# zssjh/stereo-semantic-vo

Measured on AMD Instinct MI355X. Metric: stereo frames/sec on KITTI 00 (full Tracking::Track chain), higher is better.
Workload: dtype u8; 1 GPU; BASELINE configs[2]: synth-kitti00 sequence of 4541 distinct 1241x376 stereo pairs, full Tracking::Track loop per frame (ORB on L and R, sparse stereo, matching passes 1+2, PnP-RANSAC, pose-only LM, map-point lifecycle); ONE sequence per GPU in strict frame order (replicas across GPUs); parallelism=one GPU, resident_pairs_per_gpu=4541, resident_input_bytes_per_gpu=4370984960, frames_tracked=4541, tracker_capacity_flag=0, pnp_samples_through_sequential_fallback=0

## Files before the change

stereo-semantic-vo_amd/csrc/svo_pose_dev.h:

```cpp
#pragma once
#include "svo_internal.h"
#include "svo_wave.h"

struct Se3 { double q[4]; double t[3]; };

__device__ __forceinline__ double pose_ndiv(double a, double b) {
  double r = __builtin_amdgcn_rcp(b);
  double e = __builtin_fma(-b, r, 1.0);
  r = __builtin_fma(r, e, r);
  e = __builtin_fma(-b, r, 1.0);
  r = __builtin_fma(r, e, r);
  const double q = a * r;
  const double rem = __builtin_fma(-b, q, a);
  return __builtin_fma(rem, r, q);
}
__device__ __forceinline__ double pose_rcp_refined(double b) {
  double r = __builtin_amdgcn_rcp(b);
  double e = __builtin_fma(-b, r, 1.0);
  r = __builtin_fma(r, e, r);
  e = __builtin_fma(-b, r, 1.0);
  r = __builtin_fma(r, e, r);
  return r;
}
__device__ __forceinline__ double pose_ndiv_r(double a, double b, double r) {
// ... 575 lines not shown
#include "svo_epnp_ord_dev.h"

struct PnpHyp {
  double R[9], t[3];
  int32_t cnt, ok;
};

__device__ __forceinline__ bool pnp_inlier(const double* R, const double* t, const double* X, const double* uv, const double* K) {
  double x = R[0] * X[0] + R[1] * X[1] + R[2] * X[2] + t[0];
  double y = R[3] * X[0] + R[4] * X[1] + R[5] * X[2] + t[1];
  double z = R[6] * X[0] + R[7] * X[1] + R[8] * X[2] + t[2];
  z = z != 0.0 ? 1. / z : 1.;
  x *= z; y *= z;
  const float px = (float)(x * K[0] + K[2]), py = (float)(y * K[1] + K[3]);
  const float dx = (float)uv[0] - px, dy = (float)uv[1] - py;
  const float err = dx * dx + dy * dy;
  return err <= 64.0f;
}

__device__ __forceinline__ void pnp_hyp_block(EpnpWaveLds* ws, const double* Xw, const double* uv, int n, const double* K,
                                              const uint16_t* subset, PnpHyp* out, int hyp_base) {
  const int lane = threadIdx.x & 63, wv = threadIdx.x >> 6;
  const int k = hyp_base + wv;
  if (k >= PNP_HYP) return;
  if (lane < 5) {
    const int e = min((int)subset[5 * k + lane], n - 1);
    ws[wv].x5[3 * lane] = Xw[3 * e]; ws[wv].x5[3 * lane + 1] = Xw[3 * e + 1]; ws[wv].x5[3 * lane + 2] = Xw[3 * e + 2];
    ws[wv].u5[2 * lane] = uv[2 * e]; ws[wv].u5[2 * lane + 1] = uv[2 * e + 1];
  }
  double R[9], t[3];
  const bool ok = epnp5_wave(ws[wv], K, R, t);
  int cnt = 0;
  if (ok)
    for (int e = lane; e < n; e += 64) cnt += pnp_inlier(R, t, Xw + 3 * e, uv + 2 * e, K) ? 1 : 0;
  cnt = wave_sum_i32_dpp(cnt);
  if (lane == 0) {
    PnpHyp h;
#pragma unroll
    for (int i = 0; i < 9; ++i) h.R[i] = R[i];
    h.t[0] = t[0]; h.t[1] = t[1]; h.t[2] = t[2];
    h.cnt = cnt; h.ok = ok ? 1 : 0;
    out[k] = h;
  }
}

struct PnpExactLds { epnp_exact::Work W; double R[9], t[3]; int ok; };
__device__ __forceinline__ void pnp_hyp_exact_wave(PnpExactLds& S, const double* Xw, const double* uv, int n, const double* K,
                                                   const uint16_t* subset, PnpHyp* out, int k) {
  const int lane = threadIdx.x & 63;
  if (k >= PNP_HYP) return;
  if (lane == 0) {
    double* x5 = S.W.PW0;
    double* u5 = S.W.gA;
    for (int i = 0; i < 5; ++i) {
      const int e = min((int)subset[5 * k + i], n - 1);
      x5[3 * i] = Xw[3 * e]; x5[3 * i + 1] = Xw[3 * e + 1]; x5[3 * i + 2] = Xw[3 * e + 2];
      u5[2 * i] = uv[2 * e]; u5[2 * i + 1] = uv[2 * e + 1];
    }
    S.ok = epnp_exact::solve5(S.W, x5, u5, K, S.R, S.t, nullptr) ? 1 : 0;
  }
  __builtin_amdgcn_fence(__ATOMIC_ACQ_REL, "workgroup");
  __builtin_amdgcn_wave_barrier();
  double R[9], t[3];
#pragma unroll
  for (int i = 0; i < 9; ++i) R[i] = S.R[i];
#pragma unroll
  for (int i = 0; i < 3; ++i) t[i] = S.t[i];
  const bool ok = S.ok != 0;
  int cnt = 0;
  if (ok)
    for (int e = lane; e < n; e += 64) cnt += pnp_inlier(R, t, Xw + 3 * e, uv + 2 * e, K) ? 1 : 0;
  cnt = wave_sum_i32_dpp(cnt);
  if (lane == 0) {
    PnpHyp h;
#pragma unroll
    for (int i = 0; i < 9; ++i) h.R[i] = R[i];
    h.t[0] = t[0]; h.t[1] = t[1]; h.t[2] = t[2];
    h.cnt = cnt; h.ok = ok ? 1 : 0;
    out[k] = h;
  }
}

struct PnpOrdLds { epnp_ord::Lds S; epnp_exact::Work W; };
template <bool AGENT_OUT = false>
__device__ __forceinline__ void pnp_hyp_ord_wave(PnpOrdLds& L, const double* Xw, const double* uv, int n, const double* K,
                                                 const uint16_t* subset, PnpHyp* out, int k, bool force_seq = false,
                                                 unsigned* word = nullptr ) {
  const int lane = threadIdx.x & 63;
  if (k >= PNP_HYP) return;
  if (lane < 5) {
    const int e = min((int)subset[5 * k + lane], n - 1);
    L.S.pws[3 * lane] = Xw[3 * e]; L.S.pws[3 * lane + 1] = Xw[3 * e + 1]; L.S.pws[3 * lane + 2] = Xw[3 * e + 2];
    L.S.us[2 * lane] = uv[2 * e]; L.S.us[2 * lane + 1] = uv[2 * e + 1];
  }
  double R[9], t[3];
  const bool ok = epnp_ord::solve5_wave(L.S, L.W, K, R, t, nullptr, force_seq);
  int cnt = 0;
  if (ok)
    for (int e = lane; e < n; e += 64) cnt += pnp_inlier(R, t, Xw + 3 * e, uv + 2 * e, K) ? 1 : 0;
  cnt = wave_sum_i32_dpp(cnt);
  if (lane == 0) {
    if (word) *word = (ok ? 0x80000000u : 0u) | (unsigned)cnt;
    if (AGENT_OUT) {
      PnpHyp* o = out + k;
#pragma unroll
      for (int i = 0; i < 9; ++i) __hip_atomic_store(reinterpret_cast<long long*>(&o->R[i]), __builtin_bit_cast(long long, R[i]), __ATOMIC_RELAXED, __HIP_MEMORY_SCOPE_AGENT);
#pragma unroll
      for (int i = 0; i < 3; ++i) __hip_atomic_store(reinterpret_cast<long long*>(&o->t[i]), __builtin_bit_cast(long long, t[i]), __ATOMIC_RELAXED, __HIP_MEMORY_SCOPE_AGENT);
      __hip_atomic_store(&o->cnt, cnt, __ATOMIC_RELAXED, __HIP_MEMORY_SCOPE_AGENT);
      __hip_atomic_store(&o->ok, ok ? 1 : 0, __ATOMIC_RELAXED, __HIP_MEMORY_SCOPE_AGENT);
    } else {
      PnpHyp h;
#pragma unroll
      for (int i = 0; i < 9; ++i) h.R[i] = R[i];
      h.t[0] = t[0]; h.t[1] = t[1]; h.t[2] = t[2];
      h.cnt = cnt; h.ok = ok ? 1 : 0;
      out[k] = h;
    }
  }
}

__device__ __forceinline__ int pnp_update_iters(double ep, int maxIters) {
  const double p = 0.99;
  ep = fmax(ep, 0.); ep = fmin(ep, 1.);
  double num = fmax(1. - p, 2.2250738585072014e-308);
  double denom = 1. - pow(1. - ep, 5.0);
  if (denom < 2.2250738585072014e-308) return 0;
  num = log(num);
  denom = log(denom);
  return denom >= 0 || -num >= maxIters * (-denom) ? maxIters : (int)rint(num / denom);
}

__device__ __forceinline__ int pnp_bound_after(const int* cnt, const int* ok, int n, int m) {
  int niters = PNP_HYP, maxGood = 0;
  if (n == 5) return 1;
  for (int iter = 0; iter < m && iter < niters; ++iter) {
    if (!ok[iter]) continue;
    const int g = cnt[iter];
    if (g > max(maxGood, 4)) { maxGood = g; niters = pnp_update_iters((double)(n - g) / n, niters); }
  }
  return niters;
}

__device__ __forceinline__ void pnp_update_terms(int g, int n, double* ld, int* r) {
  double ep = (double)(n - g) / n;
  ep = fmax(ep, 0.); ep = fmin(ep, 1.);
  const double denom = 1. - pow(1. - ep, 5.0);
  if (denom < 2.2250738585072014e-308) { *ld = 1.0; *r = 0; return; }
  const double num = log(fmax(1. - 0.99, 2.2250738585072014e-308));
  *ld = log(denom);
  *r = *ld < 0 ? (int)rint(num / *ld) : 0;
}
__device__ __forceinline__ int pnp_select_pre(const int* cnt, const int* ok, const double* ld, const int* r, int n, int* good, int* iters) {
  int niters = PNP_HYP, maxGood = 0, best = -1, run = 0;
  if (n == 5) {
    *good = ok[0] ? 5 : 0; *iters = 1;
    return ok[0] ? 0 : -1;
  }
  const double num = log(fmax(1. - 0.99, 2.2250738585072014e-308));
  for (int iter = 0; iter < niters; ++iter) {
    ++run;
    if (!ok[iter]) continue;
    const int g = cnt[iter];
    if (g > max(maxGood, 4)) {
      maxGood = g; best = iter;
      const double d = ld[iter];
      if (d == 1.0) niters = 0;
      else niters = d >= 0 || -num >= niters * (-d) ? niters : r[iter];
    }
  }
  *good = maxGood; *iters = run;
  return best;
}

__device__ __forceinline__ int pnp_select_pre_bound(const int* cnt, const int* ok, const double* ld, const int* r, int n, int m) {
  int niters = PNP_HYP, maxGood = 0;
  if (n == 5) return 1;
  const double num = log(fmax(1. - 0.99, 2.2250738585072014e-308));
  int iter = 0;
  for (; iter < niters; ++iter) {
    if (iter >= m) return m + 1;
    if (!ok[iter]) continue;
    const int g = cnt[iter];
    if (g > max(maxGood, 4)) {
      maxGood = g;
      const double d = ld[iter];
      if (d == 1.0) niters = 0;
      else niters = d >= 0 || -num >= niters * (-d) ? niters : r[iter];
    }
  }
  return iter;
}

__device__ __forceinline__ int pnp_select_pre_early(const int* cnt, const int* ok, const double* ld, const int* r, int n, int m,
                                                    int* best_out, int* good) {
  int niters = PNP_HYP, maxGood = 0, best = -1;
  if (n == 5) {
    *good = ok[0] ? 5 : 0; *best_out = ok[0] ? 0 : -1;
    return 1;
  }
  const double num = log(fmax(1. - 0.99, 2.2250738585072014e-308));
// ... 35 lines not shown
```

stereo-semantic-vo_amd/csrc/svo_track.hip:

```cpp
#include <chrono>
#include <cstddef>
#include <initializer_list>
#include <string>
#include <vector>
#include <algorithm>
#include <cstring>
#include <mutex>

#include "svo_internal.h"
#include "svo_wave.h"
#include "svo_gate.h"
#include "svo_pose_dev.h"
#include "svo_fmat_dev.h"

#define TRK_MAXKP 512
#define TRK_CAP 4096
#define TRK_ROWS_MAX 3072
#define TRK_LCAP 8
#define TRK_GPOS (1 << 20)
#define TRK_DNC 24
#define TRK_DENSE 0xFF

struct TrackPool {
  alignas(16) uint32_t desc[TRK_CAP * 8];
  int32_t create_id[TRK_CAP];
  int32_t gid[TRK_CAP];
  uint8_t bad[TRK_CAP];
  uint8_t in_local[TRK_CAP];
};

#define TP_EARLY 8
#define TP_FLAGS 16
struct TrackWork {
  int32_t ready;
  int32_t frame_id, nkp, n_stereo, n_pass1, n_pass2, n_new, n_local, skip_match;
  long long ts[8];
  long long rt[6];
  int32_t diag[2];
  int32_t n_edges;
  int32_t edge_gid[TRK_MAXKP];
  int32_t edge_kp[TRK_MAXKP];
  int32_t new_gid[TRK_MAXKP];
  int32_t pnp_best, pnp_iterations, pnp_inliers, pnp_ok;
  double T_pnp[16];
  int32_t hyp_done, pad_hyp;
  long long hyp_early[TP_FLAGS];
  long long hyp_rt[TP_EARLY];
};

struct TrackState {
  int32_t frame_num, npool, lastN, cur;
  int32_t next_gid, overflow, n_vetoed, n_boxes;
  int32_t epnp_fallbacks, pad_counters[3];
  int32_t last_mp[TRK_MAXKP];
  int32_t dbg_cur_mp[TRK_MAXKP];
  svo_camera cam;
  int32_t boxes[SVO_MAX_BOXES * 4];
  double F[9];
  float last_xy[TRK_MAXKP * 2];
  alignas(16) uint32_t last_desc[TRK_MAXKP * 8];
  int32_t bf_idx[TRK_MAXKP], bf_dist[TRK_MAXKP], bf_min;
  uint8_t bf_keep[TRK_MAXKP];
  float lastTcw[16];
  double Xw[TRK_MAXKP * 3], obs[TRK_MAXKP * 2], K[4], Tprior[16], T[16];
  svo_lm_stats lm;
  svo_pnp_stats pnp;
  PnpHyp hyp[PNP_HYP];
  long long pose_ts[16];
  TrackPool pool[2];
  uint16_t rowmin[TRK_CAP];
  uint8_t ncand[TRK_CAP];
  uint32_t cand[(size_t)TRK_CAP * 2 * TRK_LCAP];
  uint16_t D[(size_t)TRK_CAP * 512];
  float gpos[(size_t)TRK_GPOS * 3];
};

__device__ __forceinline__ int tk_wave_incl_scan(int v) {
  v += __builtin_amdgcn_update_dpp(0, v, 0x111, 0xf, 0xf, false);
  v += __builtin_amdgcn_update_dpp(0, v, 0x112, 0xf, 0xf, false);
  v += __builtin_amdgcn_update_dpp(0, v, 0x114, 0xf, 0xf, false);
  v += __builtin_amdgcn_update_dpp(0, v, 0x118, 0xf, 0xf, false);
  v += __builtin_amdgcn_update_dpp(0, v, 0x142, 0xa, 0xf, false);
  v += __builtin_amdgcn_update_dpp(0, v, 0x143, 0xc, 0xf, false);
  return v;
}
__device__ __forceinline__ int block_excl_scan(int v, int* sm , int* total) {
  const int lane = threadIdx.x & 63, wv = threadIdx.x >> 6;
  const int incl = tk_wave_incl_scan(v);
  const int nw = blockDim.x >> 6;
  __syncthreads();
  if (lane == 63) sm[wv] = incl;
  __syncthreads();
  const int4 a = reinterpret_cast<const int4*>(sm)[0], b = reinterpret_cast<const int4*>(sm)[1],
             c = reinterpret_cast<const int4*>(sm)[2], d = reinterpret_cast<const int4*>(sm)[3];
  const int t[16] = {a.x, a.y, a.z, a.w, b.x, b.y, b.z, b.w, c.x, c.y, c.z, c.w, d.x, d.y, d.z, d.w};
  int off = 0, tot = 0;
#pragma unroll
  for (int w = 0; w < 16; ++w) {
    off += w < wv ? t[w] : 0;
    tot += w < nw ? t[w] : 0;
  }
  *total = tot;
  return off + incl - v;
}

__device__ __forceinline__ void tk_unproject(const svo_camera& cam, float u, float v, float z,
                                             const float* Rwc, const float* twc, float* xyz) {
  const float x = (u - cam.cx) * z * (1 / cam.fx);
  const float y = (v - cam.cy) * z * (1 / cam.fy);
#pragma unroll
  for (int r = 0; r < 3; ++r) {
    const double acc = (double)Rwc[3 * r] * (double)x + (double)Rwc[3 * r + 1] * (double)y +
                       (double)Rwc[3 * r + 2] * (double)z;
    xyz[r] = (float)(acc + (double)twc[r]);
  }
}

__device__ __forceinline__ int ld_agent(const int* p) { return __hip_atomic_load(p, __ATOMIC_RELAXED, __HIP_MEMORY_SCOPE_AGENT); }
__device__ __forceinline__ long long ld_agent(const long long* p) { return __hip_atomic_load(p, __ATOMIC_RELAXED, __HIP_MEMORY_SCOPE_AGENT); }
__device__ __forceinline__ void st_agent(int* p, int v) { __hip_atomic_store(p, v, __ATOMIC_RELAXED, __HIP_MEMORY_SCOPE_AGENT); }
__device__ __forceinline__ void st_agent(long long* p, long long v) { __hip_atomic_store(p, v, __ATOMIC_RELAXED, __HIP_MEMORY_SCOPE_AGENT); }
#define TP_STORES_DONE() asm volatile("s_waitcnt vmcnt(0)" ::: "memory")
__device__ __forceinline__ long long tp_early_word(int frame_tag, unsigned ok_cnt) { return (long long)(((unsigned long long)(unsigned)frame_tag << 32) | ok_cnt); }
__device__ __forceinline__ int tp_early_tag(long long w) { return (int)((unsigned long long)w >> 32); }
__device__ __forceinline__ int tp_early_cnt(long long w) { return (int)((unsigned)w & 0x7fffffffu); }
__device__ __forceinline__ int tp_early_ok(long long w) { return (int)(((unsigned)w >> 31) & 1u); }

template <int ROWS>
__global__ __launch_bounds__(256) void k_ti_lists(TrackState* st, const uint32_t* desc, const int32_t* nkp_p, int kstride,
                                                  int lcap, int nblk) {
// ... 761 lines not shown
      if (s_lost) atomicOr(&st->overflow, 4);
    }
    __syncthreads();
    __builtin_amdgcn_fence(__ATOMIC_ACQUIRE, "agent");
    if (s_lost) return false;
  }
  return true;
}

#define TP_HYP_FIRST 16
#define TP_HYP_PRE 32
struct TpHypLds {
  double Xw[TRK_MAXKP * 3], uv[TRK_MAXKP * 2];
  EpnpWaveLds ws[4];
  int cnt[TP_HYP_PRE], ok[TP_HYP_PRE], bound;
};

__global__ __launch_bounds__(256) void k_tp_hyp(TrackState* st, const TrackWork* work, const svo_kp* kp, const uint16_t* subsets,
                                                int kstride, int hyp_base, int tag) {
  TpHypLds& S = *reinterpret_cast<TpHypLds*>(tk_smem);
  st += blockIdx.y; work += blockIdx.y; kp += (size_t)blockIdx.y * kstride;
  if (!tp_wait_work(st, work, tag)) return;
  const long long t_start = clock64();
  if (hyp_base == 0 && blockIdx.x == 0 && threadIdx.x == 0) const_cast<TrackWork*>(work)->rt[2] = wall_clock64();
  const int n = ld_agent(&work->n_edges), skip0 = ld_agent(&work->skip_match);
  const int gid0 = ld_agent(&work->edge_gid[threadIdx.x]), j0 = min(max(ld_agent(&work->edge_kp[threadIdx.x]), 0), kstride - 1);
  if (skip0 || n < 5) return;
  const int first = hyp_base + (int)blockIdx.x * (int)(blockDim.x >> 6);
  if (hyp_base > 0) {
    const int pre = min(hyp_base, TP_HYP_PRE);
    if ((int)threadIdx.x < pre) { S.cnt[threadIdx.x] = st->hyp[threadIdx.x].cnt; S.ok[threadIdx.x] = st->hyp[threadIdx.x].ok; }
    __syncthreads();
    if (threadIdx.x == 0) S.bound = pnp_bound_after(S.cnt, S.ok, n, pre);
    __syncthreads();
    if (first >= S.bound) return;
  }
  const float* gpos = st->gpos;
  for (int e = threadIdx.x; e < n; e += blockDim.x) {
    const bool first_e = e == (int)threadIdx.x;
    const float* gp = gpos + 3 * (size_t)((first_e ? gid0 : ld_agent(&work->edge_gid[e])) & (TRK_GPOS - 1));
    const svo_kp k = kp[first_e ? j0 : ld_agent(&work->edge_kp[e])];
    S.Xw[3 * e] = (double)gp[0]; S.Xw[3 * e + 1] = (double)gp[1]; S.Xw[3 * e + 2] = (double)gp[2];
    S.uv[2 * e] = (double)k.x; S.uv[2 * e + 1] = (double)k.y;
  }
  __syncthreads();
  const double K[4] = {(double)st->cam.fx, (double)st->cam.fy, (double)st->cam.cx, (double)st->cam.cy};
  const long long t_gather = clock64();
  pnp_hyp_block(S.ws, S.Xw, S.uv, n, K, subsets + (size_t)min(n, 512) * 500, st->hyp, first);
  if (first == 0 && threadIdx.x == 0) {
    st->pose_ts[0] = t_start; st->pose_ts[1] = t_gather; st->pose_ts[2] = S.ws[0].stamp[0]; st->pose_ts[3] = S.ws[0].stamp[4];
    st->pose_ts[4] = clock64();
    st->pose_ts[5] = S.ws[0].stamp[1]; st->pose_ts[6] = S.ws[0].stamp[2]; st->pose_ts[7] = S.ws[0].stamp[3]; st->pose_ts[12] = S.ws[0].sweeps;
    st->pose_ts[13] = S.ws[0].stamp[5]; st->pose_ts[14] = S.ws[0].stamp[6]; st->pose_ts[15] = S.ws[0].stamp[7];
  }
}

struct TpHypExactLds { double Xw[TRK_MAXKP * 3], uv[TRK_MAXKP * 2]; PnpExactLds ex; };
__global__ __launch_bounds__(64) void k_tp_hyp_exact(TrackState* st, TrackWork* work, const svo_kp* kp, const uint16_t* subsets,
                                                     int kstride, int tag) {
  TpHypExactLds& S = *reinterpret_cast<TpHypExactLds*>(tk_smem);
  st += blockIdx.y; work += blockIdx.y; kp += (size_t)blockIdx.y * kstride;
  if (!tp_wait_work(st, work, tag)) return;
  if (threadIdx.x == 0 && blockIdx.x == 0) work->rt[2] = wall_clock64();
  const int n = ld_agent(&work->n_edges);
  if (ld_agent(&work->skip_match) || n < 5) return;
  const float* gpos = st->gpos;
  for (int e = threadIdx.x; e < n; e += blockDim.x) {
    const float* gp = gpos + 3 * (size_t)(ld_agent(&work->edge_gid[e]) & (TRK_GPOS - 1));
    const svo_kp k = kp[ld_agent(&work->edge_kp[e])];
    S.Xw[3 * e] = (double)gp[0]; S.Xw[3 * e + 1] = (double)gp[1]; S.Xw[3 * e + 2] = (double)gp[2];
    S.uv[2 * e] = (double)k.x; S.uv[2 * e + 1] = (double)k.y;
  }
  __syncthreads();
  const double K[4] = {(double)st->cam.fx, (double)st->cam.fy, (double)st->cam.cx, (double)st->cam.cy};
  pnp_hyp_exact_wave(S.ex, S.Xw, S.uv, n, K, subsets + (size_t)min(n, 512) * 500, st->hyp, blockIdx.x);
}

struct TpHypOrdLds { double Xw[TRK_MAXKP * 3], uv[TRK_MAXKP * 2]; PnpOrdLds ord; int cnt[TP_HYP_PRE], ok[TP_HYP_PRE], bound; };
template <bool FUSED>
__device__ __forceinline__ void tp_hyp_ord_body(TpHypOrdLds& S, TrackState* st, TrackWork* work, const svo_kp* kp, const uint16_t* subsets,
                                                int kstride, int hyp_base, int sample, int tag, int force_seq, int semi = 0) {
  if (!tp_wait_work(st, work, tag)) return;
  const long long t_start = clock64();
  if (threadIdx.x == 0 && sample == 0) work->rt[2] = wall_clock64();
  const int n = ld_agent(&work->n_edges);
  const int frame_tag = FUSED ? ld_agent(&work->frame_id) + 1 : 0;
  if (ld_agent(&work->skip_match) || n < 5) return;
  if (FUSED && (force_seq >> 8) == sample + 1) return;
  if (FUSED && semi > 0) {
    const int tid = threadIdx.x;
    if (tid < semi) { S.cnt[tid] = ld_agent(&st->hyp[tid].cnt); S.ok[tid] = ld_agent(&st->hyp[tid].ok); }
    __syncthreads();
    if (tid == 0) S.bound = pnp_bound_after(S.cnt, S.ok, n, semi);
    __syncthreads();
    bool leave = sample >= S.bound;
    if (!leave && sample >= 2 * semi) {
      if (tid >= semi && tid < 2 * semi) {
        int spins = 0;
        long long w = 0;
        while (tp_early_tag(w = ld_agent(&work->hyp_early[tid])) != frame_tag && spins < (1 << 22)) { __builtin_amdgcn_s_sleep(2); ++spins; }
        const bool late = spins >= (1 << 22);
        S.cnt[tid] = late ? 0 : tp_early_cnt(w); S.ok[tid] = late ? 0 : tp_early_ok(w);
      }
      __syncthreads();
      if (tid == 0) S.bound = pnp_bound_after(S.cnt, S.ok, n, 2 * semi);
      __syncthreads();
      leave = sample >= S.bound;
    }
    if (leave) {
      if (tid == 0) {
        if (sample < TP_FLAGS) st_agent(&work->hyp_early[sample], tp_early_word(frame_tag, 0u));
        __hip_atomic_fetch_add(&work->hyp_done, 1, __ATOMIC_RELAXED, __HIP_MEMORY_SCOPE_AGENT);
      }
      return;
    }
  }
  if (hyp_base > 0) {
    const int pre = min(hyp_base, TP_HYP_PRE);
    if ((int)threadIdx.x < pre) { S.cnt[threadIdx.x] = st->hyp[threadIdx.x].cnt; S.ok[threadIdx.x] = st->hyp[threadIdx.x].ok; }
    __syncthreads();
    if (threadIdx.x == 0) S.bound = pnp_bound_after(S.cnt, S.ok, n, pre);
    __syncthreads();
    if (sample >= S.bound) return;
  }
  const float* gpos = st->gpos;
  for (int e = threadIdx.x; e < n; e += 64) {
    const float* gp = gpos + 3 * (size_t)(ld_agent(&work->edge_gid[e]) & (TRK_GPOS - 1));
    const svo_kp k = kp[ld_agent(&work->edge_kp[e])];
    S.Xw[3 * e] = (double)gp[0]; S.Xw[3 * e + 1] = (double)gp[1]; S.Xw[3 * e + 2] = (double)gp[2];
    S.uv[2 * e] = (double)k.x; S.uv[2 * e + 1] = (double)k.y;
  }
  __syncthreads();
  const double K[4] = {(double)st->cam.fx, (double)st->cam.fy, (double)st->cam.cx, (double)st->cam.cy};
  if (!FUSED && sample == 0) {
    for (int i = threadIdx.x; i < 3 * n; i += 64) st->Xw[i] = S.Xw[i];
    for (int i = threadIdx.x; i < 2 * n; i += 64) st->obs[i] = S.uv[i];
    if (threadIdx.x < 4) st->K[threadIdx.x] = K[threadIdx.x];
  }
  const long long t_gather = clock64();
  unsigned ok_cnt = 0;
  pnp_hyp_ord_wave<FUSED>(S.ord, S.Xw, S.uv, n, K, subsets + (size_t)min(n, 512) * 500, st->hyp, sample, (force_seq & 0xff) != 0, &ok_cnt);
  if (FUSED) {
    if (threadIdx.x == 0 && sample < TP_EARLY) st_agent(&work->hyp_rt[sample], (long long)wall_clock64());
    TP_STORES_DONE();
    if (threadIdx.x == 0) {
      if (sample < TP_FLAGS) st_agent(&work->hyp_early[sample], tp_early_word(frame_tag, ok_cnt));
      __hip_atomic_fetch_add(&work->hyp_done, 1, __ATOMIC_RELAXED, __HIP_MEMORY_SCOPE_AGENT);
    }
  }
  if (threadIdx.x == 0 && S.ord.S.flag) atomicAdd(&st->epnp_fallbacks, 1);
  if (sample == 0 && threadIdx.x == 0) {
    const long long* sp = S.ord.S.stamp;
    st->pose_ts[0] = t_start; st->pose_ts[1] = t_gather; st->pose_ts[2] = sp[0]; st->pose_ts[3] = sp[7];
    st->pose_ts[4] = clock64();
    st->pose_ts[5] = sp[2]; st->pose_ts[6] = sp[3]; st->pose_ts[7] = sp[4]; st->pose_ts[12] = S.ord.S.flag;
    st->pose_ts[13] = sp[4]; st->pose_ts[14] = sp[5]; st->pose_ts[15] = sp[6];
  }
}
__global__ __launch_bounds__(64) void k_tp_hyp_ord(TrackState* st, TrackWork* work, const svo_kp* kp, const uint16_t* subsets,
                                                   int kstride, int hyp_base, int tag, int force_seq) {
  TpHypOrdLds& S = *reinterpret_cast<TpHypOrdLds*>(tk_smem);
  st += blockIdx.y; work += blockIdx.y; kp += (size_t)blockIdx.y * kstride;
  tp_hyp_ord_body<false>(S, st, work, kp, subsets, kstride, hyp_base, hyp_base + (int)blockIdx.x, tag, force_seq);
}
__global__ __launch_bounds__(64) void k_tp_hyp_ord_first(TrackState* st, TrackWork* work, const svo_kp* kp, const uint16_t* subsets,
                                                         int kstride, int tag, int force_seq) {
  TpHypOrdLds& S = *reinterpret_cast<TpHypOrdLds*>(tk_smem);
  st += blockIdx.y; work += blockIdx.y; kp += (size_t)blockIdx.y * kstride;
  tp_hyp_ord_body<true>(S, st, work, kp, subsets, kstride, 0, (int)blockIdx.x, tag, force_seq);
}

struct TpLds {
  PoseLds pose;
  alignas(16) int sm[16];
  int cnt[PNP_HYP], ok[PNP_HYP], upd_r[PNP_HYP], best, good, iters;
  long long hrt[TP_EARLY];
  double tab_ld[PNP_MAXN + 1]; int tab_r[PNP_MAXN + 1];
  double pre_T[TP_EARLY][16]; Se3 pre_est[TP_EARLY];
  double T_end[16];
  long long t_samples, t_build;
  int late[TP_EARLY], lost;
  int recf[8];
  double upd_ld[PNP_HYP];
};

#define TPF_NT 256
template <bool FUSED>
__device__ __forceinline__ void tp_frame_body(TpLds& S, TrackState* st, TrackWork* work, const svo_kp* kp, const float* depth,
                                              svo_track_result* res_out, int kstride, int use_mfma, int tag, int pre_gathered) {
  const int tid = threadIdx.x;
  if (!tp_wait_work(st, work, tag)) return;
  if (!FUSED && tid == 0) work->rt[4] = wall_clock64();
  const long long tf0 = clock64();
  const int id = ld_agent(&work->frame_id), nkp = ld_agent(&work->nkp), skip = ld_agent(&work->skip_match), n_edges = ld_agent(&work->n_edges);
  const int gid0 = ld_agent(&work->edge_gid[tid]), j0 = min(max(ld_agent(&work->edge_kp[tid]), 0), kstride - 1);
  float* gpos = st->gpos;
  if (tid >= 64 && tid < 71) {
    const int* src = tid == 64 ? &work->n_stereo : tid == 65 ? &work->n_pass1 : tid == 66 ? &work->n_pass2 : tid == 67 ? &work->n_new
                   : tid == 68 ? &work->n_local : tid == 69 ? &work->diag[0] : &work->diag[1];
    S.recf[tid - 64] = ld_agent(src);
  }
  constexpr int NEWS = (TRK_MAXKP + TPF_NT - 1) / TPF_NT;
  int new_g[NEWS]; svo_kp new_k[NEWS]; float new_d[NEWS];
#pragma unroll
  for (int q = 0; q < NEWS; ++q) {
    const int j = tid + q * TPF_NT;
    new_g[q] = ld_agent(&work->new_gid[min(j, TRK_MAXKP - 1)]);
    new_k[q] = kp[min(j, kstride - 1)];
    new_d[q] = depth[min(j, kstride - 1)];
  }
  const bool have_corr = pre_gathered && !skip && n_edges >= 5 && id != 0;
  for (int e = tid; e < (have_corr ? 0 : n_edges); e += TPF_NT) {
    const int j = e == tid ? j0 : ld_agent(&work->edge_kp[e]);
    const svo_kp k = kp[j];
    float* gp = gpos + 3 * (size_t)((e == tid ? gid0 : ld_agent(&work->edge_gid[e])) & (TRK_GPOS - 1));
    float xyz[3];
    if (id == 0) {
      const float I3[9] = {1, 0, 0, 0, 1, 0, 0, 0, 1}, z3[3] = {0, 0, 0};
      tk_unproject(st->cam, k.x, k.y, depth[j], I3, z3, xyz);
      gp[0] = xyz[0]; gp[1] = xyz[1]; gp[2] = xyz[2];
    } else {
      xyz[0] = gp[0]; xyz[1] = gp[1]; xyz[2] = gp[2];
    }
    st->Xw[3 * e] = (double)xyz[0]; st->Xw[3 * e + 1] = (double)xyz[1]; st->Xw[3 * e + 2] = (double)xyz[2];
    st->obs[2 * e] = (double)k.x; st->obs[2 * e + 1] = (double)k.y;
    if (FUSED && e < POSE_CHUNK) {
      double* c5 = S.pose.tw + 5 * e;
      c5[0] = (double)xyz[0]; c5[1] = (double)xyz[1]; c5[2] = (double)xyz[2]; c5[3] = (double)k.x; c5[4] = (double)k.y;
    }
  }
  if (tid < 4 && !have_corr) st->K[tid] = (double)((const float*)&st->cam)[tid];
  const bool ran = !skip && n_edges >= 5;
  bool decided_early = false;
  double first[10] = {0, 0, 0, 0, 0, 0, 0, 0, 0, 0};
  if (FUSED) {
    if (tid < 4) S.pose.K[tid] = (double)((const float*)&st->cam)[tid];
    if (ran) {
      if (n_edges > 5)
        for (int g = 5 + tid; g <= n_edges; g += TPF_NT) {
          double ld; int r;
          pnp_update_terms(g, n_edges, &ld, &r);
          S.tab_ld[g] = ld; S.tab_r[g] = r;
        }
      if (tid >= TP_EARLY && tid < PNP_HYP) { S.cnt[tid] = 0; S.ok[tid] = 0; S.upd_ld[tid] = 1.0; S.upd_r[tid] = 0; }
    }
    __syncthreads();
    pose_edge_regs(S.pose.tw, S.pose.tw + 3, max(min(n_edges, POSE_CHUNK), 1), first, 5, 5);
  }
  if (FUSED && ran) {
    long long hp[12], hclk = 0;
    bool late = false;
    if (tid < TP_EARLY) {
      int spins = 0;
      long long w = 0;
      while (tp_early_tag(w = ld_agent(&work->hyp_early[tid])) != id + 1 && spins < (1 << 22)) { __builtin_amdgcn_s_sleep(1); ++spins; }
      late = spins >= (1 << 22);
      if (late) atomicOr(&st->overflow, 4);
      const PnpHyp& h = st->hyp[tid];
#pragma unroll
      for (int i = 0; i < 12; ++i) hp[i] = ld_agent(reinterpret_cast<const long long*>(i < 9 ? &h.R[i] : &h.t[i - 9]));
      hclk = ld_agent(&work->hyp_rt[tid]);
      S.late[tid] = late ? 1 : 0;
      const int c = late ? 0 : tp_early_cnt(w), o = late ? 0 : tp_early_ok(w);
      S.cnt[tid] = c; S.ok[tid] = o;
      const bool bound = o && c > 4 && n_edges > 5;
      const int g = min(max(c, 5), max(n_edges, 5));
      S.upd_ld[tid] = bound ? S.tab_ld[g] : 1.0; S.upd_r[tid] = bound ? S.tab_r[g] : 0;
    }
    __syncthreads();
    if (tid == 64) {
      int l = 0;
      for (int k = 0; k < TP_EARLY; ++k) l |= S.late[k];
      S.lost = l;
      int best = -1, good = 0;
      S.iters = l ? 0 : pnp_select_pre_early(S.cnt, S.ok, S.upd_ld, S.upd_r, n_edges, TP_EARLY, &best, &good);
      S.best = best; S.good = good;
    }
    if (tid < TP_EARLY) {
      double Tp[16];
#pragma unroll
      for (int q = 0; q < 16; ++q) {
        const int r = q >> 2, c = q & 3;
        Tp[q] = r == 3 ? (c == 3 ? 1.0 : 0.0) : __builtin_bit_cast(double, c == 3 ? hp[9 + r] : hp[3 * r + c]);
        S.pre_T[tid][q] = Tp[q];
      }
      Se3 e0;
      pose_start_estimate(Tp, 1, e0);
      S.pre_est[tid] = e0;
      S.hrt[tid] = late ? 0 : hclk;
    }
    __syncthreads();
    decided_early = S.lost || S.iters <= TP_EARLY;
    if (!decided_early) {
      if (tid == 0) {
        int spins = 0;
        while (ld_agent(&work->hyp_done) < PNP_HYP && spins < (1 << 22)) { __builtin_amdgcn_s_sleep(1); ++spins; }
        if (spins >= (1 << 22)) { atomicOr(&st->overflow, 4); S.lost = 1; }
      }
      __syncthreads();
    }
  } else if (tid == 0) {
    S.lost = 0;
  }
  if (FUSED && tid == 0) S.t_samples = wall_clock64();
  const bool fast = FUSED && ran && decided_early;
  if (!fast) {
    if (ran && !decided_early && !(FUSED && S.lost))
      for (int h = tid; h < PNP_HYP; h += TPF_NT) {
        const int c = FUSED ? ld_agent(&st->hyp[h].cnt) : st->hyp[h].cnt, o = FUSED ? ld_agent(&st->hyp[h].ok) : st->hyp[h].ok;
        S.cnt[h] = c; S.ok[h] = o;
        double ld = 1.0; int r = 0;
        if (o && c > 4 && n_edges > 5) pnp_update_terms(c, n_edges, &ld, &r);
        S.upd_ld[h] = ld; S.upd_r[h] = r;
      }
    __syncthreads();
    if (tid == 0) {
      int good = 0, iters = 0;
      S.best = (ran && !S.lost) ? pnp_select_pre(S.cnt, S.ok, S.upd_ld, S.upd_r, n_edges, &good, &iters) : -1;
      S.good = good; S.iters = iters;
    }
    __syncthreads();
  }
  const int tb = FUSED ? TPF_NT - 64 : 0;
  if (tid >= tb && tid < tb + 16) {
    const int q = tid - tb;
    double v;
    if (S.best >= 0) {
      const PnpHyp& h = st->hyp[S.best];
      const int r = q >> 2, c = q & 3;
      if (fast) {
        v = S.pre_T[S.best][q];
      } else if (FUSED) {
        const double* src = r == 3 ? nullptr : (c == 3 ? &h.t[r] : &h.R[3 * r + c]);
        v = src ? __builtin_bit_cast(double, ld_agent(reinterpret_cast<const long long*>(src))) : (c == 3 ? 1.0 : 0.0);
      } else {
        v = r == 3 ? (c == 3 ? 1.0 : 0.0) : (c == 3 ? h.t[r] : h.R[3 * r + c]);
      }
    } else {
      v = (double)st->lastTcw[q];
    }
    st->T[q] = v;
    work->T_pnp[q] = v;
  }
  if (tid == tb) {
    st->pnp.n_points = n_edges; st->pnp.n_inliers = S.best >= 0 ? S.good : 0; st->pnp.best_hypothesis = S.best;
    st->pnp.ok = S.best >= 0 ? 1 : 0; st->pnp.iterations = S.iters;
    work->pnp_best = S.best; work->pnp_iterations = S.iters; work->pnp_inliers = S.best >= 0 ? S.good : 0;
    work->pnp_ok = S.best >= 0 ? 1 : 0;
  }
  if (!fast) __syncthreads();
  const long long tf1 = clock64();
  int lm_iters = 0;
  const PosePrepared prep{(fast && S.best >= 0) ? &S.pre_est[S.best] : nullptr, first};
  pose_opt_block<TPF_NT>(S.pose, st->Xw, st->obs, n_edges, st->K, st->T, &st->lm, 1, use_mfma, &S.t_build, FUSED ? &prep : nullptr, S.T_end, &lm_iters);
  __syncthreads();
  const long long tf2 = clock64();
  float sT[16], sRwc[9], stwc[3];
#pragma unroll
  for (int i = 0; i < 16; ++i) sT[i] = (float)S.T_end[i];
#pragma unroll
  for (int i = 0; i < 9; ++i) sRwc[i] = sT[4 * (i % 3) + i / 3];
#pragma unroll
  for (int i = 0; i < 3; ++i) {
    const double acc = (double)sRwc[3 * i] * (double)sT[3] + (double)sRwc[3 * i + 1] * (double)sT[7] +
                       (double)sRwc[3 * i + 2] * (double)sT[11];
    stwc[i] = (float)(-acc);
  }
#pragma unroll
  for (int q = 0; q < NEWS; ++q) {
    const int g = tid + q * TPF_NT < nkp ? new_g[q] : -1;
    if (g < 0) continue;
    float xyz[3];
// ... 1209 lines not shown
```

Measured before the change: 9977 stereo frames/s.

## Publish early PnP hypotheses as self-tagged granules read in parallel by consumer

Early PnP hypothesis producers now write each rotation, translation, count word and clock as a self-validating 128-bit granule (value plus frame tag at both ends). The consumer spins on all 8x14 granules in parallel across threads instead of waiting for one flag and then serially reloading the hypothesis. This removes one flag-then-load dependency round trip. The producer also prefetches the first 128 edge indices and the subset indices before the early-exit checks, so that gather latency overlaps. In exchange it adds extra global stores and more spinning threads, and it relies on torn-read detection being correct under relaxed ordering.

```diff
diff --git a/stereo-semantic-vo_amd/csrc/svo_granule.h b/stereo-semantic-vo_amd/csrc/svo_granule.h
--- /dev/null
+++ b/stereo-semantic-vo_amd/csrc/svo_granule.h
@@ -0,0 +1,21 @@
+#pragma once
+#include <stdint.h>
+
+#if defined(__HIPCC__) || defined(__CUDACC__)
+#define SVO_GRAN_FN __host__ __device__ __forceinline__
+#else
+#define SVO_GRAN_FN static inline
+#endif
+
+#define SVO_GRAN_VALUES 13
+#define SVO_GRAN_CLOCK 13
+#define SVO_GRAN_SLOTS 16
+
+SVO_GRAN_FN void svo_granule_pack(uint32_t tag, uint64_t bits, uint64_t w[2]) {
+  w[0] = (uint64_t)tag | (bits << 32);
+  w[1] = (bits >> 32) | ((uint64_t)tag << 32);
+}
+SVO_GRAN_FN bool svo_granule_unpack(uint64_t w0, uint64_t w1, uint32_t tag, uint64_t* bits) {
+  *bits = (w0 >> 32) | (w1 << 32);
+  return tag != 0u && (uint32_t)w0 == tag && (uint32_t)(w1 >> 32) == tag;
+}
diff --git a/stereo-semantic-vo_amd/csrc/svo_pose_dev.h b/stereo-semantic-vo_amd/csrc/svo_pose_dev.h
--- a/stereo-semantic-vo_amd/csrc/svo_pose_dev.h
+++ b/stereo-semantic-vo_amd/csrc/svo_pose_dev.h
@@ -681,41 +681,37 @@
 }
 
 struct PnpOrdLds { epnp_ord::Lds S; epnp_exact::Work W; };
-template <bool AGENT_OUT = false>
-__device__ __forceinline__ void pnp_hyp_ord_wave(PnpOrdLds& L, const double* Xw, const double* uv, int n, const double* K,
-                                                 const uint16_t* subset, PnpHyp* out, int k, bool force_seq = false,
-                                                 unsigned* word = nullptr ) {
+template <bool PRE_SUB = false>
+__device__ __forceinline__ bool pnp_hyp_ord_solve(PnpOrdLds& L, const double* Xw, const double* uv, int n, const double* K,
+                                                  const uint16_t* subset, int k, bool force_seq, int sub_e, double* R, double* t, int* cnt_out) {
   const int lane = threadIdx.x & 63;
-  if (k >= PNP_HYP) return;
   if (lane < 5) {
-    const int e = min((int)subset[5 * k + lane], n - 1);
+    const int e = min(PRE_SUB ? sub_e : (int)subset[5 * k + lane], n - 1);
     L.S.pws[3 * lane] = Xw[3 * e]; L.S.pws[3 * lane + 1] = Xw[3 * e + 1]; L.S.pws[3 * lane + 2] = Xw[3 * e + 2];
     L.S.us[2 * lane] = uv[2 * e]; L.S.us[2 * lane + 1] = uv[2 * e + 1];
   }
-  double R[9], t[3];
   const bool ok = epnp_ord::solve5_wave(L.S, L.W, K, R, t, nullptr, force_seq);
   int cnt = 0;
   if (ok)
     for (int e = lane; e < n; e += 64) cnt += pnp_inlier(R, t, Xw + 3 * e, uv + 2 * e, K) ? 1 : 0;
-  cnt = wave_sum_i32_dpp(cnt);
+  *cnt_out = wave_sum_i32_dpp(cnt);
+  return ok;
+}
+template <bool PRE_SUB = false>
+__device__ __forceinline__ void pnp_hyp_ord_wave(PnpOrdLds& L, const double* Xw, const double* uv, int n, const double* K,
+                                                 const uint16_t* subset, PnpHyp* out, int k, bool force_seq = false, int sub_e = 0) {
+  const int lane = threadIdx.x & 63;
+  if (k >= PNP_HYP) return;
+  double R[9], t[3];
+  int cnt;
+  const bool ok = pnp_hyp_ord_solve<PRE_SUB>(L, Xw, uv, n, K, subset, k, force_seq, sub_e, R, t, &cnt);
   if (lane == 0) {
-    if (word) *word = (ok ? 0x80000000u : 0u) | (unsigned)cnt;
-    if (AGENT_OUT) {
-      PnpHyp* o = out + k;
-#pragma unroll
-      for (int i = 0; i < 9; ++i) __hip_atomic_store(reinterpret_cast<long long*>(&o->R[i]), __builtin_bit_cast(long long, R[i]), __ATOMIC_RELAXED, __HIP_MEMORY_SCOPE_AGENT);
-#pragma unroll
-      for (int i = 0; i < 3; ++i) __hip_atomic_store(reinterpret_cast<long long*>(&o->t[i]), __builtin_bit_cast(long long, t[i]), __ATOMIC_RELAXED, __HIP_MEMORY_SCOPE_AGENT);
-      __hip_atomic_store(&o->cnt, cnt, __ATOMIC_RELAXED, __HIP_MEMORY_SCOPE_AGENT);
-      __hip_atomic_store(&o->ok, ok ? 1 : 0, __ATOMIC_RELAXED, __HIP_MEMORY_SCOPE_AGENT);
-    } else {
-      PnpHyp h;
-#pragma unroll
-      for (int i = 0; i < 9; ++i) h.R[i] = R[i];
-      h.t[0] = t[0]; h.t[1] = t[1]; h.t[2] = t[2];
-      h.cnt = cnt; h.ok = ok ? 1 : 0;
-      out[k] = h;
-    }
+    PnpHyp h;
+#pragma unroll
+    for (int i = 0; i < 9; ++i) h.R[i] = R[i];
+    h.t[0] = t[0]; h.t[1] = t[1]; h.t[2] = t[2];
+    h.cnt = cnt; h.ok = ok ? 1 : 0;
+    out[k] = h;
   }
 }
 
diff --git a/stereo-semantic-vo_amd/csrc/svo_track.hip b/stereo-semantic-vo_amd/csrc/svo_track.hip
--- a/stereo-semantic-vo_amd/csrc/svo_track.hip
+++ b/stereo-semantic-vo_amd/csrc/svo_track.hip
@@ -11,6 +11,7 @@
 #include "svo_wave.h"
 #include "svo_gate.h"
 #include "svo_pose_dev.h"
+#include "svo_granule.h"
 #include "svo_fmat_dev.h"
 
 #define TRK_MAXKP 512
@@ -46,6 +47,7 @@
   int32_t hyp_done, pad_hyp;
   long long hyp_early[TP_FLAGS];
   long long hyp_rt[TP_EARLY];
+  alignas(128) long long gran[TP_EARLY][2 * SVO_GRAN_SLOTS];
 };
 
 struct TrackState {
@@ -973,11 +975,17 @@
                                                 int kstride, int hyp_base, int sample, int tag, int force_seq, int semi = 0) {
   if (!tp_wait_work(st, work, tag)) return;
   const long long t_start = clock64();
-  if (threadIdx.x == 0 && sample == 0) work->rt[2] = wall_clock64();
+  const int lane = threadIdx.x;
   const int n = ld_agent(&work->n_edges);
   const int frame_tag = FUSED ? ld_agent(&work->frame_id) + 1 : 0;
-  if (ld_agent(&work->skip_match) || n < 5) return;
+  const int skip0 = ld_agent(&work->skip_match);
+  int gid01[2], j01[2];
+#pragma unroll
+  for (int q = 0; q < 2; ++q) { gid01[q] = ld_agent(&work->edge_gid[lane + 64 * q]); j01[q] = ld_agent(&work->edge_kp[lane + 64 * q]); }
+  if (threadIdx.x == 0 && sample == 0) work->rt[2] = wall_clock64();
+  if (skip0 || n < 5) return;
   if (FUSED && (force_seq >> 8) == sample + 1) return;
+  if (sample == 0 && threadIdx.x == 0) st->pose_ts[12] = clock64();
   if (FUSED && semi > 0) {
     const int tid = threadIdx.x;
     if (tid < semi) { S.cnt[tid] = ld_agent(&st->hyp[tid].cnt); S.ok[tid] = ld_agent(&st->hyp[tid].ok); }
@@ -1015,11 +1023,29 @@
     if (sample >= S.bound) return;
   }
   const float* gpos = st->gpos;
-  for (int e = threadIdx.x; e < n; e += 64) {
+  const int sub_e = lane < 5 ? (int)subsets[(size_t)min(n, 512) * 500 + 5 * sample + lane] : 0;
+  float px[2][3], kxy[2][2];
+#pragma unroll
+  for (int q = 0; q < 2; ++q) {
+    const float* gp = gpos + 3 * (size_t)(gid01[q] & (TRK_GPOS - 1));
+    const svo_kp* k = kp + min(max(j01[q], 0), kstride - 1);
+    px[q][0] = gp[0]; px[q][1] = gp[1]; px[q][2] = gp[2];
+    kxy[q][0] = k->x; kxy[q][1] = k->y;
+  }
+#pragma unroll
+  for (int q = 0; q < 2; ++q) {
+    const int e = lane + 64 * q;
+    if (e < n) {
+      S.Xw[3 * e] = (double)px[q][0]; S.Xw[3 * e + 1] = (double)px[q][1]; S.Xw[3 * e + 2] = (double)px[q][2];
+      S.uv[2 * e] = (double)kxy[q][0]; S.uv[2 * e + 1] = (double)kxy[q][1];
+    }
+  }
+  for (int e = lane + 128; e < n; e += 64) {
     const float* gp = gpos + 3 * (size_t)(ld_agent(&work->edge_gid[e]) & (TRK_GPOS - 1));
-    const svo_kp k = kp[ld_agent(&work->edge_kp[e])];
-    S.Xw[3 * e] = (double)gp[0]; S.Xw[3 * e + 1] = (double)gp[1]; S.Xw[3 * e + 2] = (double)gp[2];
-    S.uv[2 * e] = (double)k.x; S.uv[2 * e + 1] = (double)k.y;
+    const svo_kp* k = kp + ld_agent(&work->edge_kp[e]);
+    const float x0 = gp[0], x1 = gp[1], x2 = gp[2], u = k->x, v = k->y;
+    S.Xw[3 * e] = (double)x0; S.Xw[3 * e + 1] = (double)x1; S.Xw[3 * e + 2] = (double)x2;
+    S.uv[2 * e] = (double)u; S.uv[2 * e + 1] = (double)v;
   }
   __syncthreads();
   const double K[4] = {(double)st->cam.fx, (double)st->cam.fy, (double)st->cam.cx, (double)st->cam.cy};
@@ -1029,22 +1055,49 @@
     if (threadIdx.x < 4) st->K[threadIdx.x] = K[threadIdx.x];
   }
   const long long t_gather = clock64();
-  unsigned ok_cnt = 0;
-  pnp_hyp_ord_wave<FUSED>(S.ord, S.Xw, S.uv, n, K, subsets + (size_t)min(n, 512) * 500, st->hyp, sample, (force_seq & 0xff) != 0, &ok_cnt);
   if (FUSED) {
-    if (threadIdx.x == 0 && sample < TP_EARLY) st_agent(&work->hyp_rt[sample], (long long)wall_clock64());
+    double R[9], t[3];
+    int cnt;
+    const bool ok = pnp_hyp_ord_solve<true>(S.ord, S.Xw, S.uv, n, K, nullptr, sample, (force_seq & 0xff) != 0, sub_e, R, t, &cnt);
+    const unsigned ok_cnt = (ok ? 0x80000000u : 0u) | (unsigned)cnt;
+    if (sample < TP_EARLY) {
+      unsigned long long bits = (unsigned long long)ok_cnt;
+#pragma unroll
+      for (int i = 0; i < 9; ++i) bits = lane == i ? __builtin_bit_cast(unsigned long long, R[i]) : bits;
+#pragma unroll
+      for (int i = 0; i < 3; ++i) bits = lane == 9 + i ? __builtin_bit_cast(unsigned long long, t[i]) : bits;
+      uint64_t w[2];
+      if (lane < SVO_GRAN_VALUES) {
+        svo_granule_pack((uint32_t)frame_tag, bits, w);
+        st_agent(&work->gran[sample][2 * lane], (long long)w[0]); st_agent(&work->gran[sample][2 * lane + 1], (long long)w[1]);
+      }
+      const long long clk = (long long)wall_clock64();
+      if (lane == SVO_GRAN_CLOCK) {
+        svo_granule_pack((uint32_t)frame_tag, (uint64_t)clk, w);
+        st_agent(&work->gran[sample][2 * lane], (long long)w[0]); st_agent(&work->gran[sample][2 * lane + 1], (long long)w[1]);
+      }
+      if (lane == 0) st_agent(&work->hyp_rt[sample], clk);
+    }
+    if (lane == 0) {
+      PnpHyp* o = st->hyp + sample;
+#pragma unroll
+      for (int i = 0; i < 9; ++i) st_agent(reinterpret_cast<long long*>(&o->R[i]), __builtin_bit_cast(long long, R[i]));
+#pragma unroll
+      for (int i = 0; i < 3; ++i) st_agent(reinterpret_cast<long long*>(&o->t[i]), __builtin_bit_cast(long long, t[i]));
+      st_agent(&o->cnt, cnt); st_agent(&o->ok, ok ? 1 : 0);
+      if (sample < TP_FLAGS) st_agent(&work->hyp_early[sample], tp_early_word(frame_tag, ok_cnt));
+    }
     TP_STORES_DONE();
-    if (threadIdx.x == 0) {
-      if (sample < TP_FLAGS) st_agent(&work->hyp_early[sample], tp_early_word(frame_tag, ok_cnt));
-      __hip_atomic_fetch_add(&work->hyp_done, 1, __ATOMIC_RELAXED, __HIP_MEMORY_SCOPE_AGENT);
-    }
+    if (lane == 0) __hip_atomic_fetch_add(&work->hyp_done, 1, __ATOMIC_RELAXED, __HIP_MEMORY_SCOPE_AGENT);
+  } else {
+    pnp_hyp_ord_wave<true>(S.ord, S.Xw, S.uv, n, K, nullptr, st->hyp, sample, (force_seq & 0xff) != 0, sub_e);
   }
   if (threadIdx.x == 0 && S.ord.S.flag) atomicAdd(&st->epnp_fallbacks, 1);
   if (sample == 0 && threadIdx.x == 0) {
     const long long* sp = S.ord.S.stamp;
     st->pose_ts[0] = t_start; st->pose_ts[1] = t_gather; st->pose_ts[2] = sp[0]; st->pose_ts[3] = sp[7];
     st->pose_ts[4] = clock64();
-    st->pose_ts[5] = sp[2]; st->pose_ts[6] = sp[3]; st->pose_ts[7] = sp[4]; st->pose_ts[12] = S.ord.S.flag;
+    st->pose_ts[5] = sp[2]; st->pose_ts[6] = sp[3]; st->pose_ts[7] = sp[4];
     st->pose_ts[13] = sp[4]; st->pose_ts[14] = sp[5]; st->pose_ts[15] = sp[6];
   }
 }
@@ -1126,6 +1179,7 @@
   double first[10] = {0, 0, 0, 0, 0, 0, 0, 0, 0, 0};
   if (FUSED) {
     if (tid < 4) S.pose.K[tid] = (double)((const float*)&st->cam)[tid];
+    if (tid < TP_EARLY) S.late[tid] = 0;
     if (ran) {
       if (n_edges > 5)
         for (int g = 5 + tid; g <= n_edges; g += TPF_NT) {
@@ -1139,24 +1193,29 @@
     pose_edge_regs(S.pose.tw, S.pose.tw + 3, max(min(n_edges, POSE_CHUNK), 1), first, 5, 5);
   }
   if (FUSED && ran) {
-    long long hp[12], hclk = 0;
-    bool late = false;
-    if (tid < TP_EARLY) {
+    if (tid < 16 * TP_EARLY && (tid & 15) <= SVO_GRAN_CLOCK) {
+      const int k = tid >> 4, i = tid & 15;
+      const long long* g = &work->gran[k][2 * i];
       int spins = 0;
-      long long w = 0;
-      while (tp_early_tag(w = ld_agent(&work->hyp_early[tid])) != id + 1 && spins < (1 << 22)) { __builtin_amdgcn_s_sleep(1); ++spins; }
-      late = spins >= (1 << 22);
-      if (late) atomicOr(&st->overflow, 4);
-      const PnpHyp& h = st->hyp[tid];
-#pragma unroll
-      for (int i = 0; i < 12; ++i) hp[i] = ld_agent(reinterpret_cast<const long long*>(i < 9 ? &h.R[i] : &h.t[i - 9]));
-      hclk = ld_agent(&work->hyp_rt[tid]);
-      S.late[tid] = late ? 1 : 0;
-      const int c = late ? 0 : tp_early_cnt(w), o = late ? 0 : tp_early_ok(w);
-      S.cnt[tid] = c; S.ok[tid] = o;
-      const bool bound = o && c > 4 && n_edges > 5;
-      const int g = min(max(c, 5), max(n_edges, 5));
-      S.upd_ld[tid] = bound ? S.tab_ld[g] : 1.0; S.upd_r[tid] = bound ? S.tab_r[g] : 0;
+      uint64_t bits = 0;
+      while (!svo_granule_unpack((uint64_t)ld_agent(g), (uint64_t)ld_agent(g + 1), (uint32_t)(id + 1), &bits) && spins < (1 << 22)) { __builtin_amdgcn_s_sleep(1); ++spins; }
+      const bool late = spins >= (1 << 22);
+      if (late) { atomicOr(&st->overflow, 4); S.late[k] = 1; }
+      if (i < 12) {
+        S.pre_T[k][i < 9 ? 4 * (i / 3) + i % 3 : 4 * (i - 9) + 3] = __builtin_bit_cast(double, bits);
+      } else if (i == 12) {
+        const long long w = (long long)bits;
+        const int c = late ? 0 : tp_early_cnt(w), o = late ? 0 : tp_early_ok(w);
+        S.cnt[k] = c; S.ok[k] = o;
+        const bool bound = o && c > 4 && n_edges > 5;
+        const int gg = min(max(c, 5), max(n_edges, 5));
+        S.upd_ld[k] = bound ? S.tab_ld[gg] : 1.0; S.upd_r[k] = bound ? S.tab_r[gg] : 0;
+      } else {
+        S.hrt[k] = late ? 0 : (long long)bits;
+      }
+    } else if (tid >= 16 * TP_EARLY && tid < 16 * TP_EARLY + 4 * TP_EARLY) {
+      const int q = tid - 16 * TP_EARLY;
+      S.pre_T[q >> 2][12 + (q & 3)] = (q & 3) == 3 ? 1.0 : 0.0;
     }
     __syncthreads();
     if (tid == 64) {
@@ -1170,15 +1229,10 @@
     if (tid < TP_EARLY) {
       double Tp[16];
 #pragma unroll
-      for (int q = 0; q < 16; ++q) {
-        const int r = q >> 2, c = q & 3;
-        Tp[q] = r == 3 ? (c == 3 ? 1.0 : 0.0) : __builtin_bit_cast(double, c == 3 ? hp[9 + r] : hp[3 * r + c]);
-        S.pre_T[tid][q] = Tp[q];
-      }
+      for (int q = 0; q < 16; ++q) Tp[q] = S.pre_T[tid][q];
       Se3 e0;
       pose_start_estimate(Tp, 1, e0);
       S.pre_est[tid] = e0;
-      S.hrt[tid] = late ? 0 : hclk;
     }
     __syncthreads();
     decided_early = S.lost || S.iters <= TP_EARLY;
```

Result: no change. 10040 stereo frames/s, median of 6 (+0.6%).
